# terrense/TTS-sambert_hifiGAN

Hardware: AMD Instinct MI355X
Metric: audio samples/sec/GPU (HiFi-GAN 80-mel→22.05 kHz) at 1/2/4/8 MI355X; RTF (higher is better)
Workload: dtype f16x3

## Files before the change

### profiles/ab_show.py

```python
import json
import os
import sys

tag = sys.argv[1] if len(sys.argv) > 1 else "ab"
out = os.environ.get("OUT_DIR", "profiles/out")
for f in ("new1", "old1", "new2", "old2"):
    d = json.loads(open(f"{out}/{tag}_{f}.json").read().strip().splitlines()[-1])
    ks = {k.split("(")[0][:34]: round(v["ms_per_step"], 3) for k, v in d["kernels"].items()
          if v["ms_per_step"] > 0.1}
    print(f, round(d["ms_per_step"], 3), ks)
```

### tts-sambert_hifigan_amd/csrc/ups_bf16x3.hip

```cpp
#include <hip/hip_runtime.h>

#include <cstdio>

#include "bf16x3_common.h"
#include "kernels.h"
#include "launch.h"

#ifndef HFG_UPS_PAIR
#define HFG_UPS_PAIR 1
#endif

#ifndef HFG_UPS_SMALL_OCC
#define HFG_UPS_SMALL_OCC 3
#endif

namespace hfg {

template <int WAVES_M, int WAVES_N, int WM, int WN>
constexpr int ups_min_blocks() { return WAVES_M * WM * WN <= 2 ? HFG_UPS_SMALL_OCC : 2; }

template <int WAVES_M, int WAVES_N, int WM, int WN, int NP, int FMT>
__global__ void __launch_bounds__(64 * WAVES_M * WAVES_N, (ups_min_blocks<WAVES_M, WAVES_N, WM, WN>()))
ups_bf16x3(const UpsParams p) {
  constexpr int NW = WAVES_M * WAVES_N;
  constexpr int MT = 32 * WM * WAVES_M;
  constexpr int NTILE = 32 * WN * WAVES_N;
  constexpr UpsLds LY = ups_lds(UpsCfg{WAVES_M, WAVES_N, WM, WN});
  static_assert(LY.total <= (int)kMaxLdsBytes, "LDS");
  constexpr int XR = LY.xr;
  constexpr int NQ = XR / 4;
  constexpr int NTASK = 2 * NQ;
  constexpr int TPW = (NTASK + NW - 1) / NW;
  static_assert(TPW <= 64, "one staging task per lane");
  constexpr int XPLANE = LY.xplane;
  constexpr int XBUF = LY.xbuf;
  constexpr int SLAB = LY.slab;
  constexpr int PW = SLAB / 1024 / NW;
  static_assert(PW * 1024 * NW == SLAB, "slab must split evenly over the waves");

  auto xrow_off = [](int r, int h) {
    return 16 * ((2 * r + h) ^ (((r >> 3) & 1) * 5 + ((r >> 2) & 1) * 2));
  };
  extern __shared__ __attribute__((aligned(16))) char lds[];
  char* const Abuf = lds;
  char* const Xbuf = lds + LY.x_off;

  const int tid = threadIdx.x;
  const int lane = tid & 63;
  const int wave = __builtin_amdgcn_readfirstlane(tid >> 6);
  const int wave_m = wave % WAVES_M;
  const int wave_n = wave / WAVES_M;
  const int half = lane >> 5;
  const int col = lane & 31;

  int mt, tx, b;
  {
    const int total = p.m_tiles * p.n_tiles * p.batch;
    int id = blockIdx.x;
    const int q = total >> 3;
    if (id < (q << 3)) id = (id & 7) * q + (id >> 3);
    mt = id % p.m_tiles;
    id /= p.m_tiles;
    tx = id % p.n_tiles;
    b = id / p.n_tiles;
    mt = __builtin_amdgcn_readfirstlane(mt);
    tx = __builtin_amdgcn_readfirstlane(tx);
    b = __builtin_amdgcn_readfirstlane(b);
  }
  const int T_b = p.len_in ? min(p.len_in[b], p.T) : p.T;
  const int ex = FMT == kFmtF16 ? x3_exp_slot(p.amax_in, b) : 0;
  const float sx = FMT == kFmtF16 ? exp2i(ex) : 1.0f;
  const int m0 = tx * NTILE;
  if (m0 >= T_b) return;
  const int NG = p.C_in / 16;

  const char* wsrc = reinterpret_cast<const char*>(p.w) + (int64_t)mt * NG * SLAB;
  auto issue_a = [&](int g, int slot) {
    const char* src = wsrc + (int64_t)g * SLAB;
    char* dst = Abuf + slot * SLAB;
#pragma unroll
    for (int q = 0; q < PW; ++q) {
      const int i = wave + q * NW;
      __builtin_amdgcn_global_load_lds((gptr_t1)(src + i * 1024 + lane * 16),
                                       (lds_ptr_t3)(dst + i * 1024), 16, 0, 0);
    }
  };

  const char* xb = reinterpret_cast<const char*>(p.x + (int64_t)b * p.x_bs);
  const int64_t grp_bytes = (int64_t)16 * p.L * 4;
  const int grp_rec = (int)(unsigned)(grp_bytes < 0xFFFFFFFFll ? grp_bytes : 0xFFFFFFFFll);
  const int task = wave * TPW + lane;
  const bool has_task = lane < TPW && task < NTASK;
  const int hf = task & 1;
  const int xq = task >> 1;
  const int t0 = m0 - 4 + 4 * xq;
  const float sx1 = kLReluSlope * sx;
  bool okt[4];
#pragma unroll
  for (int tt = 0; tt < 4; ++tt) okt[tt] = has_task && (unsigned)(t0 + tt) < (unsigned)T_b;
  const bool q_in = has_task && t0 >= 0 && t0 < p.L;
  const unsigned xoff_lane = q_in ? (unsigned)(8 * hf * p.L + t0) * 4u : 0u;
  const int xcs4 = p.L * 4;
  typedef float f4 __attribute__((ext_vector_type(4)));
  f4 xv[8];
  auto load_x = [&](int g) {
    const __amdgpu_buffer_rsrc_t xrs =
        __builtin_amdgcn_make_buffer_rsrc((void*)(xb + g * grp_bytes), 0, grp_rec, 0x00020000);
#pragma unroll
    for (int e = 0; e < 8; ++e)
      xv[e] = __builtin_bit_cast(
          f4, __builtin_amdgcn_raw_buffer_load_b128(xrs, (int)xoff_lane, e * xcs4, 0));
  };
  auto store_x = [&](int buf) {
    if (!has_task) return;
    char* xh = Xbuf + buf * XBUF;
#pragma unroll
    for (int j = 0; j < 4; ++j) {
      bf16x8 hv, lv;
#pragma unroll
      for (int e = 0; e < 8; e += 2) {
        floatx2_ a;
        a[0] = okt[j] ? fmaxf(xv[e][j] * sx, xv[e][j] * sx1) : 0.f;
        a[1] = okt[j] ? fmaxf(xv[e + 1][j] * sx, xv[e + 1][j] * sx1) : 0.f;
        bf16x2_ hh, ll;
        split2<FMT>(a, hh, ll);
        hv[e] = hh[0];
        hv[e + 1] = hh[1];
        lv[e] = ll[0];
        lv[e + 1] = ll[1];
      }
      const int off = xrow_off(4 * xq + j, hf);
      *reinterpret_cast<bf16x8*>(xh + off) = hv;
      *reinterpret_cast<bf16x8*>(xh + XPLANE + off) = lv;
    }
  };

  floatx16 acc[2][WM][WN];
#pragma unroll
  for (int c = 0; c < 2; ++c)
#pragma unroll
    for (int i = 0; i < WM; ++i)
#pragma unroll
      for (int k = 0; k < WN; ++k)
#pragma unroll
        for (int r = 0; r < 16; ++r) acc[c][i][k][r] = 0.f;

  issue_a(0, 0);
  load_x(0);
  store_x(0);
  wait_vm<0>();
  lds_barrier();

  const int colw = wave_n * 32 * WN + col + 4;
  for (int g = 0; g < NG; ++g) {
    const bool more = g + 1 < NG;
    const bool slab0 = kAblate && (p.dbg & 131072);
    if (more) {
      if (!slab0) issue_a(g + 1, (g + 1) & 1);
      if (!(kAblate && (p.dbg & 1024))) load_x(g + 1);
    }
    const char* as = Abuf + (slab0 ? 0 : (g & 1)) * SLAB;
    bf16x8 a[2][2][2][WM];
#pragma unroll
    for (int c = 0; c < 2; ++c)
#pragma unroll
      for (int tp = 0; tp < 2; ++tp)
#pragma unroll
        for (int pl = 0; pl < 2; ++pl)
#pragma unroll
          for (int i = 0; i < WM; ++i)
            a[c][tp][pl][i] = *reinterpret_cast<const bf16x8*>(
                as + ((((c * 2 + tp) * 2 + pl) * WAVES_M + wave_m) * WM + i) * 1024 + lane * 16);
    const char* xh = Xbuf + (g & 1) * XBUF;
    prio_mfma();
#pragma unroll
    for (int k = 0; k < WN; ++k) {
      bf16x8 bh[3], bl[3];
#pragma unroll
      for (int o = 0; o < 3; ++o) {
        const int off = xrow_off(colw + 32 * k + o - 1, half);
        bh[o] = *reinterpret_cast<const bf16x8*>(xh + off);
        bl[o] = *reinterpret_cast<const bf16x8*>(xh + XPLANE + off);
      }
#pragma unroll
      for (int i = 0; i < WM; ++i)
#pragma unroll
        for (int c = 0; c < 2; ++c)
#pragma unroll
          for (int tp = 0; tp < 2; ++tp) {
            const int o = c + tp;
            mma3<NP, FMT>(a[c][tp][0][i], a[c][tp][1][i], bh[o], bl[o], acc[c][i][k]);
          }
    }
    prio_other();
    if (more && !(kAblate && (p.dbg & 512))) store_x((g + 1) & 1);
    wait_vm<0>();
    lds_barrier();
  }

  const float sc = FMT == kFmtF16 ? exp2i(-(ex + p.ew)) : 1.0f;

  float* yb = p.y + (int64_t)b * p.y_bs;
  float vmax = 0.f;
  auto t2 = [&](float a, float c) { vmax = fmaxf(vmax, fmaxf(fabsf(a), fabsf(c))); };
  const int h = p.u >> 1;
#pragma unroll
  for (int i = 0; i < WM; ++i) {
    const int rb = mt * MT + wave_m * 32 * WM + i * 32 + 4 * half;
#pragma unroll
    for (int k = 0; k < WN; ++k) {
      const int m = m0 + wave_n * 32 * WN + k * 32 + col;
      if (m >= T_b) continue;
      if (h == 1 && HFG_UPS_PAIR) {
        const bool odd = col & 1;
        const int me = m - (odd ? 1 : 0);
        const bool quad_ok = me + 1 < T_b;
#pragma unroll
        for (int r = 0; r < 16; r += 2) {
          const int co0 = rb + acc_row(r);
          const float b0 = p.bias[co0], b1 = p.bias[co0 + 1];
          const float l0 = __builtin_fmaf(acc[0][i][k][r], sc, b0);
          const float r0 = __builtin_fmaf(acc[1][i][k][r], sc, b0);
          const float l1 = __builtin_fmaf(acc[0][i][k][r + 1], sc, b1);
          const float r1 = __builtin_fmaf(acc[1][i][k][r + 1], sc, b1);
          const float s0 = odd ? l0 : l1, s1 = odd ? r0 : r1;
          const float v0 = __builtin_bit_cast(
              float, __builtin_amdgcn_mov_dpp(__builtin_bit_cast(int, s0), 0xB1, 0xF, 0xF, false));
          const float v1 = __builtin_bit_cast(
              float, __builtin_amdgcn_mov_dpp(__builtin_bit_cast(int, s1), 0xB1, 0xF, 0xF, false));
          if (quad_ok) {
            float4 v;
            v.x = odd ? v0 : l0;
            v.y = odd ? v1 : r0;
            v.z = odd ? l1 : v0;
            v.w = odd ? r1 : v1;
            if (!(kAblate && (p.dbg & 262144))) *reinterpret_cast<float4*>(yb + (int64_t)(odd ? co0 + 1 : co0) * p.L_out + 2 * me) = v;
            t2(v.x, v.y);
            t2(v.z, v.w);
          } else {
            floatx2_ a, c;
            a[0] = l0;
            a[1] = r0;
            c[0] = l1;
            c[1] = r1;
            if (!(kAblate && (p.dbg & 262144))) *reinterpret_cast<floatx2_*>(yb + (int64_t)co0 * p.L_out + 2 * m) = a;
            if (!(kAblate && (p.dbg & 262144))) *reinterpret_cast<floatx2_*>(yb + (int64_t)(co0 + 1) * p.L_out + 2 * m) = c;
            t2(l0, r0);
            t2(l1, r1);
          }
        }
      } else if (h == 1) {
#pragma unroll
        for (int r = 0; r < 16; ++r) {
          const int co = rb + acc_row(r);
          const float bv = p.bias[co];
          floatx2_ v;
          v[0] = __builtin_fmaf(acc[0][i][k][r], sc, bv);
          v[1] = __builtin_fmaf(acc[1][i][k][r], sc, bv);
          if (!(kAblate && (p.dbg & 262144))) *reinterpret_cast<floatx2_*>(yb + (int64_t)co * p.L_out + 2 * m) = v;
          t2(v[0], v[1]);
        }
      } else if (h == 2) {
#pragma unroll
        for (int q = 0; q < 4; ++q)
#pragma unroll
          for (int pr = 0; pr < 2; ++pr) {
            const int r0 = 4 * q + 2 * pr;
            const int co = (rb + 8 * q + 2 * pr) >> 1;
            const float bv = p.bias[co];
            float4 v;
            v.x = __builtin_fmaf(acc[0][i][k][r0], sc, bv);
            v.y = __builtin_fmaf(acc[0][i][k][r0 + 1], sc, bv);
            v.z = __builtin_fmaf(acc[1][i][k][r0], sc, bv);
            v.w = __builtin_fmaf(acc[1][i][k][r0 + 1], sc, bv);
            if (!(kAblate && (p.dbg & 262144))) *reinterpret_cast<float4*>(yb + (int64_t)co * p.L_out + 4 * m) = v;
            t2(v.x, v.y);
            t2(v.z, v.w);
          }
      } else {
#pragma unroll
        for (int q = 0; q < 4; ++q) {
          const int row = rb + 8 * q;
          const int co = row / h, sp = row - co * h;
          const float bv = p.bias[co];
#pragma unroll
          for (int c = 0; c < 2; ++c) {
            float4 v;
            v.x = __builtin_fmaf(acc[c][i][k][4 * q + 0], sc, bv);
            v.y = __builtin_fmaf(acc[c][i][k][4 * q + 1], sc, bv);
            v.z = __builtin_fmaf(acc[c][i][k][4 * q + 2], sc, bv);
            v.w = __builtin_fmaf(acc[c][i][k][4 * q + 3], sc, bv);
            if (!(kAblate && (p.dbg & 262144))) *reinterpret_cast<float4*>(yb + (int64_t)co * p.L_out + m * p.u + c * h + sp) = v;
            t2(v.x, v.y);
            t2(v.z, v.w);
          }
        }
      }
    }
  }
  if (p.amax_out) amax_commit(vmax, p.amax_out, b);
}

namespace {

struct EntryUps {
  int cfg, np, fmt;
  Instance<UpsParams> inst;
};

#define HFGUPS_ENTRY(CFG, NP, FMT)                                                    \
  {                                                                                   \
    CFG, NP, FMT, {                                                                   \
      ups_bf16x3<kUpsCfgs[CFG].WAVES_M, kUpsCfgs[CFG].WAVES_N, kUpsCfgs[CFG].WM,      \
                 kUpsCfgs[CFG].WN, NP, FMT>,                                          \
          {0}                                                                         \
    }                                                                                 \
  }

EntryUps g_entriesUps[] = {HFGUPS_ENTRY(0, 3, 0), HFGUPS_ENTRY(1, 3, 0), HFGUPS_ENTRY(0, 3, 1),
                           HFGUPS_ENTRY(1, 3, 1), HFGUPS_ENTRY(0, 2, 1), HFGUPS_ENTRY(1, 2, 1)};

}

size_t ups_lds_bytes(int cfg) { return (size_t)ups_lds(kUpsCfgs[cfg]).total; }

hipError_t launch_ups_bf16x3(int cfg, int fmt, int np, const UpsParams& p, hipStream_t stream,
                             const char** name) {
  EntryUps* e = nullptr;
  for (auto& cand : g_entriesUps)
    if (cand.cfg == cfg && cand.np == np && cand.fmt == fmt) e = &cand;
  if (!e) return hipErrorInvalidValue;
  const UpsCfg& t = kUpsCfgs[cfg];
  if (p.C_in % 16 != 0 || p.L % 4 != 0 || p.T > p.L || p.u < 2 || (p.u & 1) ||
      !ups_rate_ok(p.u) || p.L_out < p.L * p.u || p.m_tiles * t.MT() * 2 != p.C_out * p.u ||
      p.n_tiles * t.NTILE() < p.T || (int64_t)p.C_in * p.L > ((int64_t)1 << 30))
    return hipErrorInvalidValue;
  auto fmt_name = [&](char* s, size_t n) {
    snprintf(s, n, "ups_bf16x3<%d, %d, %d, %d, %d, %d>", t.WAVES_M, t.WAVES_N, t.WM, t.WN, np, fmt);
  };
  const int blocks = p.m_tiles * p.n_tiles * p.batch;
  return launch_instance(e->inst, fmt_name, dim3(blocks), dim3(t.threads()), ups_lds_bytes(cfg),
                         stream, name, p);
}

}
```

Before: 156.9 million.

## Redistribute upsample X staging to one quad-quarter per lane and hoist bias loads

Changes the X-tile staging in the upsampling transposed-conv kernel so every lane of every wave handles one (4-frame quad, 4-channel quarter) sub-task. Before, the tasks were 8-channel halves packed onto the first lanes of each wave. This halves the per-lane register footprint for staged X, spreads the global loads across all lanes, and uses 8-byte LDS writes, with wave 0 loading the two halo frames separately. It also hoists the bias loads out of the WN loop into a per-WM register array so the epilogue stops reloading bias per column tile. The tradeoffs are more, smaller LDS writes with possible bank-conflict changes, plus extra halo-handling logic that depends on NTILE == 64*NW.

```diff
diff --git a/profiles/ab_show.py b/profiles/ab_show.py
--- a/profiles/ab_show.py
+++ b/profiles/ab_show.py
@@ -1,11 +1,22 @@
+import glob
+import hashlib
 import json
 import os
+import re
 import sys
 
 tag = sys.argv[1] if len(sys.argv) > 1 else "ab"
 out = os.environ.get("OUT_DIR", "profiles/out")
-for f in ("new1", "old1", "new2", "old2"):
-    d = json.loads(open(f"{out}/{tag}_{f}.json").read().strip().splitlines()[-1])
-    ks = {k.split("(")[0][:34]: round(v["ms_per_step"], 3) for k, v in d["kernels"].items()
+files = sorted(glob.glob(f"{out}/{tag}_old*.json") + glob.glob(f"{out}/{tag}_new*.json"),
+               key=lambda f: (int(re.search(r"(\d+)\.json$", f).group(1)), "new" in os.path.basename(f)))
+for f in files:
+    d = json.loads(open(f).read().strip().splitlines()[-1])
+    ks = {k.split("(")[0][:34]: round(v["ms_per_step"], 4) for k, v in d.get("kernels", {}).items()
           if v["ms_per_step"] > 0.1}
-    print(f, round(d["ms_per_step"], 3), ks)
+    sums = {"main": d.get("wav_checksum32")}
+    sums.update({p: a.get("wav_checksum32") for p, a in (d.get("alt") or {}).items()
+                 if isinstance(a, dict)})
+    wav = f[:-5] + "/wav.npy"
+    sha = hashlib.sha256(open(wav, "rb").read()).hexdigest()[:16] if os.path.exists(wav) else None
+    print(os.path.basename(f)[len(tag) + 1:-5], "value", round(d.get("value", 0) / 1e6, 2),
+          "ms", round(d["ms_per_step"], 4), "sums", sums, "wav.npy", sha, ks)
diff --git a/profiles/ups_staging_ab/lds_banks_b64.py b/profiles/ups_staging_ab/lds_banks_b64.py
--- /dev/null
+++ b/profiles/ups_staging_ab/lds_banks_b64.py
@@ -0,0 +1,50 @@
+import importlib.util
+import os
+
+_p = os.path.join(os.path.dirname(os.path.abspath(__file__)), "..", "..", "tests", "tools",
+                  "ups_lds_banks.py")
+_spec = importlib.util.spec_from_file_location("ups_lds_banks", _p)
+base = importlib.util.module_from_spec(_spec)
+_spec.loader.exec_module(base)
+
+WRITE64_GROUPS = [list(range(16 * g, 16 * g + 16)) for g in range(4)]
+
+
+def extra_cycles(addrs, groups, window, slot):
+    tot = 0
+    for g in groups:
+        slots = {}
+        for l in g:
+            a = addrs.get(l)
+            if a is None:
+                continue
+            slots.setdefault((a % window) // slot, set()).add(a // slot)
+        if slots:
+            tot += max(len(v) for v in slots.values()) - 1
+    return tot
+
+
+def simulate_quarters(f, NTILE=256, NW=4):
+    assert NTILE == 64 * NW
+    extra = instr = 0
+    for wave in range(NW):
+        for j in range(4):
+            addrs = {}
+            for lane in range(64):
+                cq, xq = lane & 3, 1 + wave * 16 + (lane >> 2)
+                addrs[lane] = f(4 * xq + j, cq >> 1) + 8 * (cq & 1)
+            extra += extra_cycles(addrs, WRITE64_GROUPS, 128, 8)
+            instr += 1
+    halo = {lane: f(NTILE + 4 if lane & 8 else 3, (lane & 7) >> 2) + 4 * (lane & 3)
+            for lane in range(16)}
+    h_extra = extra_cycles(halo, [list(range(32)), list(range(32, 64))], 128, 4)
+    return extra / instr, h_extra
+
+
+if __name__ == "__main__":
+    w8, hx = simulate_quarters(base.kernel_layout)
+    print(f"(quad, quarter) 8-B sub-tasks on all 64 lanes: ds_write_b64 extra/instr {w8:.2f}, "
+          f"halo write extra {hx}")
+    for cfg, kw in (("cfg 0", dict(WAVES_M=2, WN=4)), ("cfg 1", dict(WAVES_M=1, WN=2))):
+        _, r = base.simulate(base.kernel_layout, interleave=True, **kw)
+        print(f"B reads, {cfg}: extra/instr {r:.2f}")
diff --git a/tts-sambert_hifigan_amd/csrc/ups_bf16x3.hip b/tts-sambert_hifigan_amd/csrc/ups_bf16x3.hip
--- a/tts-sambert_hifigan_amd/csrc/ups_bf16x3.hip
+++ b/tts-sambert_hifigan_amd/csrc/ups_bf16x3.hip
@@ -27,11 +27,8 @@
   constexpr int NTILE = 32 * WN * WAVES_N;
   constexpr UpsLds LY = ups_lds(UpsCfg{WAVES_M, WAVES_N, WM, WN});
   static_assert(LY.total <= (int)kMaxLdsBytes, "LDS");
-  constexpr int XR = LY.xr;
-  constexpr int NQ = XR / 4;
-  constexpr int NTASK = 2 * NQ;
-  constexpr int TPW = (NTASK + NW - 1) / NW;
-  static_assert(TPW <= 64, "one staging task per lane");
+  static_assert(LY.xr == NTILE + 8, "staged frames: [m0 - 4, m0 + NTILE + 4)");
+  static_assert(NTILE == 64 * NW, "one (quad, 4-channel quarter) staging sub-task per lane");
   constexpr int XPLANE = LY.xplane;
   constexpr int XBUF = LY.xbuf;
   constexpr int SLAB = LY.slab;
@@ -89,36 +86,46 @@
   const char* xb = reinterpret_cast<const char*>(p.x + (int64_t)b * p.x_bs);
   const int64_t grp_bytes = (int64_t)16 * p.L * 4;
   const int grp_rec = (int)(unsigned)(grp_bytes < 0xFFFFFFFFll ? grp_bytes : 0xFFFFFFFFll);
-  const int task = wave * TPW + lane;
-  const bool has_task = lane < TPW && task < NTASK;
-  const int hf = task & 1;
-  const int xq = task >> 1;
+  const int cq = lane & 3;
+  const int hf = cq >> 1;
+  const int xq = 1 + wave * 16 + (lane >> 2);
   const int t0 = m0 - 4 + 4 * xq;
   const float sx1 = kLReluSlope * sx;
   bool okt[4];
 #pragma unroll
-  for (int tt = 0; tt < 4; ++tt) okt[tt] = has_task && (unsigned)(t0 + tt) < (unsigned)T_b;
-  const bool q_in = has_task && t0 >= 0 && t0 < p.L;
-  const unsigned xoff_lane = q_in ? (unsigned)(8 * hf * p.L + t0) * 4u : 0u;
+  for (int tt = 0; tt < 4; ++tt) okt[tt] = (unsigned)(t0 + tt) < (unsigned)T_b;
+  const bool q_in = t0 < p.L;
+  const unsigned xoff_lane = q_in ? (unsigned)(4 * cq * p.L + t0) * 4u : 0u;
   const int xcs4 = p.L * 4;
+  const int hcp = lane & 7;
+  const int hrow = lane & 8 ? NTILE + 4 : 3;
+  const int ht = m0 - 4 + hrow;
+  const bool hok = (unsigned)ht < (unsigned)T_b;
+  const unsigned hoff_lane = hok ? (unsigned)(2 * hcp * p.L + ht) * 4u : 0u;
   typedef float f4 __attribute__((ext_vector_type(4)));
-  f4 xv[8];
+  f4 xv[4];
+  float hx[2];
   auto load_x = [&](int g) {
     const __amdgpu_buffer_rsrc_t xrs =
         __builtin_amdgcn_make_buffer_rsrc((void*)(xb + g * grp_bytes), 0, grp_rec, 0x00020000);
 #pragma unroll
-    for (int e = 0; e < 8; ++e)
+    for (int e = 0; e < 4; ++e)
       xv[e] = __builtin_bit_cast(
           f4, __builtin_amdgcn_raw_buffer_load_b128(xrs, (int)xoff_lane, e * xcs4, 0));
+    if (wave == 0) {
+#pragma unroll
+      for (int e = 0; e < 2; ++e)
+        hx[e] = __builtin_bit_cast(
+            float, __builtin_amdgcn_raw_buffer_load_b32(xrs, (int)hoff_lane, e * xcs4, 0));
+    }
   };
   auto store_x = [&](int buf) {
-    if (!has_task) return;
     char* xh = Xbuf + buf * XBUF;
 #pragma unroll
     for (int j = 0; j < 4; ++j) {
-      bf16x8 hv, lv;
-#pragma unroll
-      for (int e = 0; e < 8; e += 2) {
+      bf16x4_ hv, lv;
+#pragma unroll
+      for (int e = 0; e < 4; e += 2) {
         floatx2_ a;
         a[0] = okt[j] ? fmaxf(xv[e][j] * sx, xv[e][j] * sx1) : 0.f;
         a[1] = okt[j] ? fmaxf(xv[e + 1][j] * sx, xv[e + 1][j] * sx1) : 0.f;
@@ -129,9 +136,19 @@
         lv[e] = ll[0];
         lv[e + 1] = ll[1];
       }
-      const int off = xrow_off(4 * xq + j, hf);
-      *reinterpret_cast<bf16x8*>(xh + off) = hv;
-      *reinterpret_cast<bf16x8*>(xh + XPLANE + off) = lv;
+      const int off = xrow_off(4 * xq + j, hf) + 8 * (cq & 1);
+      *reinterpret_cast<bf16x4_*>(xh + off) = hv;
+      *reinterpret_cast<bf16x4_*>(xh + XPLANE + off) = lv;
+    }
+    if (wave == 0 && lane < 16) {
+      floatx2_ a;
+      a[0] = hok ? fmaxf(hx[0] * sx, hx[0] * sx1) : 0.f;
+      a[1] = hok ? fmaxf(hx[1] * sx, hx[1] * sx1) : 0.f;
+      bf16x2_ hh, ll;
+      split2<FMT>(a, hh, ll);
+      const int off = xrow_off(hrow, hcp >> 2) + 4 * (hcp & 3);
+      *reinterpret_cast<bf16x2_*>(xh + off) = hh;
+      *reinterpret_cast<bf16x2_*>(xh + XPLANE + off) = ll;
     }
   };
 
@@ -207,6 +224,17 @@
 #pragma unroll
   for (int i = 0; i < WM; ++i) {
     const int rb = mt * MT + wave_m * 32 * WM + i * 32 + 4 * half;
+    float bvr[16];
+    if (h == 1) {
+#pragma unroll
+      for (int r = 0; r < 16; ++r) bvr[r] = p.bias[rb + acc_row(r)];
+    } else if (h == 2) {
+#pragma unroll
+      for (int q = 0; q < 8; ++q) bvr[q] = p.bias[(rb + 8 * (q >> 1) + 2 * (q & 1)) >> 1];
+    } else {
+#pragma unroll
+      for (int q = 0; q < 4; ++q) bvr[q] = p.bias[(rb + 8 * q) / h];
+    }
 #pragma unroll
     for (int k = 0; k < WN; ++k) {
       const int m = m0 + wave_n * 32 * WN + k * 32 + col;
@@ -218,7 +246,7 @@
 #pragma unroll
         for (int r = 0; r < 16; r += 2) {
           const int co0 = rb + acc_row(r);
-          const float b0 = p.bias[co0], b1 = p.bias[co0 + 1];
+          const float b0 = bvr[r], b1 = bvr[r + 1];
           const float l0 = __builtin_fmaf(acc[0][i][k][r], sc, b0);
           const float r0 = __builtin_fmaf(acc[1][i][k][r], sc, b0);
           const float l1 = __builtin_fmaf(acc[0][i][k][r + 1], sc, b1);
@@ -253,7 +281,7 @@
 #pragma unroll
         for (int r = 0; r < 16; ++r) {
           const int co = rb + acc_row(r);
-          const float bv = p.bias[co];
+          const float bv = bvr[r];
           floatx2_ v;
           v[0] = __builtin_fmaf(acc[0][i][k][r], sc, bv);
           v[1] = __builtin_fmaf(acc[1][i][k][r], sc, bv);
@@ -267,7 +295,7 @@
           for (int pr = 0; pr < 2; ++pr) {
             const int r0 = 4 * q + 2 * pr;
             const int co = (rb + 8 * q + 2 * pr) >> 1;
-            const float bv = p.bias[co];
+            const float bv = bvr[2 * q + pr];
             float4 v;
             v.x = __builtin_fmaf(acc[0][i][k][r0], sc, bv);
             v.y = __builtin_fmaf(acc[0][i][k][r0 + 1], sc, bv);
@@ -282,7 +310,7 @@
         for (int q = 0; q < 4; ++q) {
           const int row = rb + 8 * q;
           const int co = row / h, sp = row - co * h;
-          const float bv = p.bias[co];
+          const float bv = bvr[q];
 #pragma unroll
           for (int c = 0; c < 2; ++c) {
             float4 v;
```

New measurement: 159.5 million, median of 6. 1.02x the previous value.
